# wyf0912/ContextGS

Measured on AMD Instinct MI355X. Metric: views/sec fwd+bwd @1920×1080, 1M anchors, higher is better.
Workload: dtype f32

## Files before the change

contextgs_amd/csrc/mlp3.hip:

```cpp
#include "cgs_internal.h"
#include "mlp_frag.h"
#include "buf_access.h"

#define M3_IN 54
#define M3_HID 50
#define M3_NTI 4
#define M3_XP 64
#define M3_NT1 4
#define M3_HP 64
#define M3_HCAT 150
#define M3_HLD 150
#define M3_HPITCH 50
#define M3_GLD 192
#define M3_GPITCH 64
#define M3_XLD 54
#ifndef M3_FWD_RT
#define M3_FWD_RT 1
#define M3_FWD_WAVES 16
#endif
#define M3_FWD_PATCH (16 * 70)
#ifndef M3_BWD_RT
#define M3_BWD_RT 2
#define M3_BWD_WAVES 8
#endif

#define M3_FENCE()                         \
    do {                                   \
        asm volatile("" ::: "memory");     \
        __builtin_amdgcn_sched_barrier(0); \
    } while (0)

struct M3Head {
    const float *W1, *b1, *W2, *b2;
    float *Y;
    const float *dY;
    float *dZ2;
};

template <int OUT>
struct M3FwdLds {
    static constexpr int NT2 = (OUT + 15) / 16, OP = NT2 * 16;
    static constexpr int S1 = frag_pad4mod8(M3_HP), S2 = frag_pad4mod8(OP);
    static constexpr int FLOATS = M3_XP * S1 + M3_HP * S2 + M3_HP + OP;
};

template <int OUT>
__device__ __forceinline__ void m3_stage_fwd(float *lds, const M3Head &h, int tid, int nthr) {
    using L = M3FwdLds<OUT>;
    float *W1s = lds, *W2s = W1s + M3_XP * L::S1, *b1s = W2s + M3_HP * L::S2, *b2s = b1s + M3_HP;
    frag_stage_transposed<M3_IN, M3_HID, M3_XP, L::S1>(W1s, h.W1, tid, nthr);
    frag_stage_transposed<M3_HID, OUT, M3_HP, L::S2>(W2s, h.W2, tid, nthr);
    for (int i = tid; i < M3_HP; i += nthr) b1s[i] = i < M3_HID ? h.b1[i] : 0.f;
    for (int i = tid; i < L::OP; i += nthr) b2s[i] = i < OUT ? h.b2[i] : 0.f;
}

#define M3_MAX_ROWS (4ll << 20)
struct M3FwdBufs { ClBuf H, Y[3], Xo, X, src, feat, anc; };

template <int OUT, int ACT, int RT, bool TILED, bool TM>
__device__ __forceinline__ void m3_head_fwd(const float *lds, const M3Head &h, int head, const f32x4 (&xb)[RT][M3_NTI],
                                            const bool (&valid)[RT], int64_t row0, int g, int c,
                                            float *__restrict__ Hcat, const M3FwdBufs &B, float *patch) {
    using L = M3FwdLds<OUT>;
    const float *W1s = lds, *W2s = W1s + M3_XP * L::S1, *b1s = W2s + M3_HP * L::S2, *b2s = b1s + M3_HP;
    f32x4 acc1[M3_NT1][RT];
#pragma unroll
    for (int t = 0; t < M3_NT1; ++t)
#pragma unroll
        for (int rt = 0; rt < RT; ++rt) acc1[t][rt] = (f32x4){0.f, 0.f, 0.f, 0.f};
#pragma unroll
    for (int q = 0; q < M3_NTI; ++q)
#pragma unroll
        for (int j = 0; j < 4; ++j) {
            if (16 * q + j >= M3_IN) continue;
            if (TM && q == M3_NTI - 1 && 16 * q + 4 * j >= M3_IN) continue;
#pragma unroll
            for (int t = 0; t < M3_NT1; ++t) {
                const float a = W1s[((TM && q == M3_NTI - 1) ? 16 * q + g + 4 * j : 16 * q + 4 * g + j) * L::S1 + 16 * t + c];
#pragma unroll
                for (int rt = 0; rt < RT; ++rt) acc1[t][rt] = frag_mfma(a, xb[rt][q][j], acc1[t][rt]);
            }
        }
#pragma unroll
    for (int t = 0; t < M3_NT1; ++t)
#pragma unroll
        for (int rt = 0; rt < RT; ++rt) {
            const int64_t row = row0 + rt * 16 + c;
#pragma unroll
            for (int r = 0; r < 4; ++r) acc1[t][rt][r] = fmaxf(acc1[t][rt][r] + b1s[16 * t + 4 * g + r], 0.f);
            if (TILED)
                frag_tstore4<M3_HID>(B.H, (uint32_t)((row0 + rt * 16) >> 4) * (16 * M3_HLD * 4) + (uint32_t)head * (16 * M3_HID * 4), t, g, c,
                                     valid[rt], acc1[t][rt]);
            else
                frag_bstore4<M3_HID>(B.H, (uint32_t)row * (M3_HLD * 4) + (uint32_t)(M3_HPITCH * head) * 4, t, g, valid[rt], acc1[t][rt]);
        }
    f32x4 acc2[L::NT2][RT];
#pragma unroll
    for (int u = 0; u < L::NT2; ++u)
#pragma unroll
        for (int rt = 0; rt < RT; ++rt) acc2[u][rt] = (f32x4){0.f, 0.f, 0.f, 0.f};
#pragma unroll
    for (int t = 0; t < M3_NT1; ++t)
#pragma unroll
        for (int r = 0; r < 4; ++r) {
            if (16 * t + r >= M3_HID) continue;
#pragma unroll
            for (int u = 0; u < L::NT2; ++u) {
                const float a = W2s[(16 * t + 4 * g + r) * L::S2 + 16 * u + c];
#pragma unroll
                for (int rt = 0; rt < RT; ++rt) acc2[u][rt] = frag_mfma(a, acc1[t][rt][r], acc2[u][rt]);
            }
        }
#pragma unroll
    for (int rt = 0; rt < RT; ++rt) {
        f32x4 yv[L::NT2];
#pragma unroll
        for (int u = 0; u < L::NT2; ++u)
#pragma unroll
            for (int r = 0; r < 4; ++r) yv[u][r] = frag_act<ACT>(acc2[u][rt][r] + b2s[16 * u + 4 * g + r]);
        frag_tile_store<OUT, L::NT2>(patch, B.Y[head], (uint32_t)(row0 + rt * 16) * (OUT * 4), yv, g, c, 16 * g + c);
    }
}

struct M3Rows {
    const float *feat_src;
    const int64_t *src_row;
    const float *anchor;
    const float *cam;
    float *X_out;
    float *d_feat_src;
    float *d_anchor;
};

template <bool TM = false>
__device__ __forceinline__ f32x4 m3_load_x_rows_b(const M3FwdBufs &B, float cam0, float cam1, float cam2, int64_t row, int64_t srow,
                                                  int q, int g, bool valid) {
    const uint32_t fo = (uint32_t)srow * (M3_HID * 4);
    if (q < 3) return cl_l128(B.feat, cl_sel(valid, fo + (uint32_t)(16 * q + 4 * g) * 4));
    if (TM) {
        const f32x4 f2 = cl_l64(B.feat, cl_sel(valid && g < 2, fo + 48 * 4));
        const f32x4 a = cl_l96(B.anc, cl_sel(valid, (uint32_t)row * 12));
        const float ux = a[0] - cam0, uy = a[1] - cam1, uz = a[2] - cam2;
        const float dist = sqrtf(ux * ux + uy * uy + uz * uz);
        const float s0 = g == 0 ? f2[0] : (g == 1 ? f2[1] : (g == 2 ? ux / dist : uy / dist));
        const float s1 = g == 0 ? uz / dist : (g == 1 ? dist : 0.f);
        return valid ? (f32x4){s0, s1, 0.f, 0.f} : (f32x4){0.f, 0.f, 0.f, 0.f};
    }
    const f32x4 f2 = cl_l64(B.feat, cl_sel(valid && g == 0, fo + 48 * 4));
    const f32x4 a = cl_l96(B.anc, cl_sel(valid && g < 2, (uint32_t)row * 12));
    const float ux = a[0] - cam0, uy = a[1] - cam1, uz = a[2] - cam2;
    const float dist = sqrtf(ux * ux + uy * uy + uz * uz);
    const f32x4 v0 = (f32x4){f2[0], f2[1], ux / dist, uy / dist}, v1 = (f32x4){uz / dist, dist, 0.f, 0.f};
    const f32x4 z = (f32x4){0.f, 0.f, 0.f, 0.f};
    return !valid ? z : (g == 0 ? v0 : (g == 1 ? v1 : z));
}

template <int O0, int A0, int O1, int A1, int O2, int A2, int RT, int WAVES, bool ROWS, bool TILED = false>
__global__ void __launch_bounds__(WAVES * 64)
    mlp3_fwd_kernel(const float *__restrict__ X, int64_t ldx, M3Head h0, M3Head h1, M3Head h2,
                    float *__restrict__ Hcat, int64_t n, M3Rows R) {
    constexpr int WFL = M3FwdLds<O0>::FLOATS + M3FwdLds<O1>::FLOATS + M3FwdLds<O2>::FLOATS;
    static_assert(WFL % 4 == 0 && O0 <= 70 && O1 <= 70 && O2 <= 70 && M3_IN <= 70, "patch: 16-byte aligned, the widest image fits");
    __shared__ __attribute__((aligned(16))) float lds[WFL + WAVES * M3_FWD_PATCH];
    float *l0 = lds, *l1 = l0 + M3FwdLds<O0>::FLOATS, *l2 = l1 + M3FwdLds<O1>::FLOATS;
    const int tid = threadIdx.x, nthr = WAVES * 64;
    float *patch = lds + WFL + (tid >> 6) * M3_FWD_PATCH;
    m3_stage_fwd<O0>(l0, h0, tid, nthr);
    m3_stage_fwd<O1>(l1, h1, tid, nthr);
    m3_stage_fwd<O2>(l2, h2, tid, nthr);
    __syncthreads();
    const int lane = tid & 63, wave = tid >> 6, g = lane >> 4, c = lane & 15;
    const int64_t ntiles = (n + 16 * RT - 1) / (16 * RT);
    f32x4 xb[RT][M3_NTI], xn[RT][M3_NTI];
    bool valid[RT], validn[RT];
    const int64_t tile0 = (int64_t)blockIdx.x * WAVES + wave, tstride = (int64_t)gridDim.x * WAVES;
    M3FwdBufs B;
    {
        const uint64_t nb = (uint64_t)n;
        const uint64_t nbt = (nb + 15) / 16 * 16;
        B.H = cl_buf(Hcat, (TILED ? nbt : nb) * (M3_HLD * 4));
        B.Y[0] = cl_buf(h0.Y, nb * (O0 * 4)); B.Y[1] = cl_buf(h1.Y, nb * (O1 * 4)); B.Y[2] = cl_buf(h2.Y, nb * (O2 * 4));
        B.Xo = cl_buf(ROWS ? R.X_out : nullptr, nb * (M3_XLD * 4));
        B.X = cl_buf(ROWS ? nullptr : X, nb > 0 ? ((nb - 1) * (uint64_t)ldx + M3_IN) * 4 : 0);
        B.src = cl_buf(ROWS ? R.src_row : nullptr, nb * 8);
        B.feat = cl_buf(ROWS ? R.feat_src : nullptr, CL_MAX_BYTES);
        B.anc = cl_buf(ROWS ? R.anchor : nullptr, nb * 12);
    }
    const float cam0 = ROWS ? R.cam[0] : 0.f, cam1 = ROWS ? R.cam[1] : 0.f, cam2 = ROWS ? R.cam[2] : 0.f;
    const uint32_t ldx4 = (uint32_t)ldx * 4;
    int64_t srow_n[RT], srow_nn[RT];
#pragma unroll
    for (int rt = 0; rt < RT; ++rt) {
        const int64_t row = tile0 * 16 * RT + rt * 16 + c, rown = row + tstride * 16 * RT;
        valid[rt] = tile0 < ntiles && row < n;
        const int64_t srow = ROWS ? cl_li64(B.src, cl_sel(valid[rt], (uint32_t)row * 8)) : 0;
        srow_n[rt] = ROWS ? cl_li64(B.src, cl_sel(rown < n, (uint32_t)rown * 8)) : 0;
#pragma unroll
        for (int q = 0; q < M3_NTI; ++q)
            xb[rt][q] = ROWS ? m3_load_x_rows_b<true>(B, cam0, cam1, cam2, row, srow, q, g, valid[rt])
                             : frag_bmask4<M3_IN>(frag_bload4<M3_IN>(B.X, (uint32_t)row * ldx4, q, g, valid[rt]), q, g);
    }
    for (int64_t tile = tile0; tile < ntiles; tile += tstride) {
        const int64_t row0 = tile * 16 * RT;
        asm volatile("" ::: "memory");
#pragma unroll
        for (int rt = 0; rt < RT; ++rt) {
            const int64_t row = (tile + tstride) * 16 * RT + rt * 16 + c, rownn = row + tstride * 16 * RT;
            validn[rt] = row < n;
            srow_nn[rt] = ROWS ? cl_li64(B.src, cl_sel(rownn < n, (uint32_t)rownn * 8)) : 0;
#pragma unroll
            for (int q = 0; q < M3_NTI; ++q)
                xn[rt][q] = ROWS ? m3_load_x_rows_b<true>(B, cam0, cam1, cam2, row, srow_n[rt], q, g, validn[rt])
                                 : frag_bmask4<M3_IN>(frag_bload4<M3_IN>(B.X, (uint32_t)row * ldx4, q, g, validn[rt]), q, g);
        }
        if (ROWS) {
#pragma unroll
            for (int rt = 0; rt < RT; ++rt)
                if (R.X_out) {
#pragma unroll
                    for (int q = 0; q < M3_NTI - 1; ++q) cl_patch_put4(patch + c * M3_IN + 16 * q + 4 * g, xb[rt][q], 4);
                    patch[c * M3_IN + 48 + g] = xb[rt][M3_NTI - 1][0];
                    if (g < 2) patch[c * M3_IN + 52 + g] = xb[rt][M3_NTI - 1][1];
                    cl_patch_flush<64 * M3_IN>(patch, B.Xo, (uint32_t)(row0 + rt * 16) * (M3_XLD * 4), lane);
                }
        }
        m3_head_fwd<O0, A0, RT, TILED, ROWS>(l0, h0, 0, xb, valid, row0, g, c, Hcat, B, patch);
        m3_head_fwd<O1, A1, RT, TILED, ROWS>(l1, h1, 1, xb, valid, row0, g, c, Hcat, B, patch);
        m3_head_fwd<O2, A2, RT, TILED, ROWS>(l2, h2, 2, xb, valid, row0, g, c, Hcat, B, patch);
#pragma unroll
        for (int rt = 0; rt < RT; ++rt) {
            valid[rt] = validn[rt];
            srow_n[rt] = srow_nn[rt];
#pragma unroll
            for (int q = 0; q < M3_NTI; ++q) xb[rt][q] = xn[rt][q];
        }
    }
}

template <int OUT>
struct M3BwdLds {
    static constexpr int NT2 = (OUT + 15) / 16, OP = NT2 * 16;
    static constexpr int SA = frag_pad4mod8(M3_HP), SB = frag_pad4mod8(M3_XP);
    static constexpr int FLOATS = OP * SA + M3_HP * SB;
};

template <int OUT>
__device__ __forceinline__ void m3_stage_bwd(float *lds, const M3Head &h, int tid, int nthr) {
    using L = M3BwdLds<OUT>;
    float *W2n = lds, *W1n = W2n + L::OP * L::SA;
    frag_stage_loop(h.W2, L::OP * L::SA, tid, nthr,
                    [](int i) { const int o = i / L::SA, hh = i % L::SA; return (o < OUT && hh < M3_HID) ? o * M3_HID + hh : -1; },
                    [&](int i, float v) { W2n[i] = v; });
    frag_stage_loop(h.W1, M3_HP * L::SB, tid, nthr,
                    [](int i) { const int hh = i / L::SB, k = i % L::SB; return (hh < M3_HID && k < M3_IN) ? hh * M3_IN + k : -1; },
                    [&](int i, float v) { W1n[i] = v; });
}

template <int OUT, int ACT, int RT>
__device__ __forceinline__ void m3_head_bwd(const float *lds, const M3Head &h, int head, const bool (&valid)[RT],
                                            int64_t row0, int g, int c, const float *__restrict__ Hcat,
                                            float *__restrict__ dZ1cat, f32x4 (&adx)[M3_NTI][RT]) {
    using L = M3BwdLds<OUT>;
    const float *W2n = lds, *W1n = W2n + L::OP * L::SA;
    f32x4 adh[M3_NT1][RT];
#pragma unroll
    for (int t = 0; t < M3_NT1; ++t)
#pragma unroll
        for (int rt = 0; rt < RT; ++rt) adh[t][rt] = (f32x4){0.f, 0.f, 0.f, 0.f};
    f32x4 b[L::NT2][RT], yv[L::NT2][RT], hv[M3_NT1][RT];
#pragma unroll
    for (int u = 0; u < L::NT2; ++u)
#pragma unroll
        for (int rt = 0; rt < RT; ++rt) {
            const int64_t row = row0 + rt * 16 + c;
            b[u][rt] = frag_load4<OUT>(h.dY + row * OUT, u, g, valid[rt]);
            if (ACT != FRAG_ACT_NONE) yv[u][rt] = frag_load4<OUT>(h.Y + row * OUT, u, g, valid[rt]);
        }
#pragma unroll
    for (int t = 0; t < M3_NT1; ++t)
#pragma unroll
        for (int rt = 0; rt < RT; ++rt)
            hv[t][rt] = frag_load4<M3_HID>(Hcat + (row0 + rt * 16 + c) * M3_HLD + M3_HPITCH * head, t, g, valid[rt]);
    if (ACT != FRAG_ACT_NONE) {
#pragma unroll
        for (int u = 0; u < L::NT2; ++u)
#pragma unroll
            for (int rt = 0; rt < RT; ++rt) {
#pragma unroll
                for (int r = 0; r < 4; ++r) b[u][rt][r] *= frag_act_grad<ACT>(yv[u][rt][r]);
                frag_store4<OUT>(h.dZ2 + (row0 + rt * 16 + c) * OUT, u, g, valid[rt], b[u][rt]);
            }
    }
#pragma unroll
    for (int u = 0; u < L::NT2; ++u)
#pragma unroll
        for (int j = 0; j < 4; ++j) {
            if (16 * u + j >= OUT) continue;
#pragma unroll
            for (int t = 0; t < M3_NT1; ++t) {
                const float a = W2n[(16 * u + 4 * g + j) * L::SA + 16 * t + c];
#pragma unroll
                for (int rt = 0; rt < RT; ++rt) adh[t][rt] = frag_mfma(a, b[u][rt][j], adh[t][rt]);
            }
        }
#pragma unroll
    for (int t = 0; t < M3_NT1; ++t)
#pragma unroll
        for (int rt = 0; rt < RT; ++rt) {
            const int64_t at = (row0 + rt * 16 + c) * M3_GLD + M3_GPITCH * head;
#pragma unroll
            for (int r = 0; r < 4; ++r) adh[t][rt][r] = hv[t][rt][r] > 0.f ? adh[t][rt][r] : 0.f;
            frag_store4<M3_HP>(dZ1cat + at, t, g, valid[rt], adh[t][rt]);
        }
#pragma unroll
    for (int t = 0; t < M3_NT1; ++t)
#pragma unroll
        for (int r = 0; r < 4; ++r) {
            if (16 * t + r >= M3_HID) continue;
#pragma unroll
            for (int v = 0; v < M3_NTI; ++v) {
                const float a = W1n[(16 * t + 4 * g + r) * L::SB + 16 * v + c];
#pragma unroll
                for (int rt = 0; rt < RT; ++rt) adx[v][rt] = frag_mfma(a, adh[t][rt][r], adx[v][rt]);
            }
        }
}

template <int O0, int A0, int O1, int A1, int O2, int A2, int RT, int WAVES, bool ROWS>
__global__ void __launch_bounds__(WAVES * 64)
    mlp3_bwd_kernel(M3Head h0, M3Head h1, M3Head h2, const float *__restrict__ Hcat, float *__restrict__ dZ1cat,
                    float *__restrict__ dX, int64_t lddx, int64_t n, M3Rows R) {
    __shared__ float lds[M3BwdLds<O0>::FLOATS + M3BwdLds<O1>::FLOATS + M3BwdLds<O2>::FLOATS];
    float *l0 = lds, *l1 = l0 + M3BwdLds<O0>::FLOATS, *l2 = l1 + M3BwdLds<O1>::FLOATS;
    const int tid = threadIdx.x, nthr = WAVES * 64;
    m3_stage_bwd<O0>(l0, h0, tid, nthr);
    m3_stage_bwd<O1>(l1, h1, tid, nthr);
    m3_stage_bwd<O2>(l2, h2, tid, nthr);
    __syncthreads();
    const int lane = tid & 63, wave = tid >> 6, g = lane >> 4, c = lane & 15;
    const int64_t ntiles = (n + 16 * RT - 1) / (16 * RT);
    for (int64_t tile = (int64_t)blockIdx.x * WAVES + wave; tile < ntiles; tile += (int64_t)gridDim.x * WAVES) {
        const int64_t row0 = tile * 16 * RT;
        asm volatile("" ::: "memory");
        bool valid[RT];
#pragma unroll
        for (int rt = 0; rt < RT; ++rt) valid[rt] = row0 + rt * 16 + c < n;
        f32x4 adx[M3_NTI][RT];
#pragma unroll
        for (int v = 0; v < M3_NTI; ++v)
#pragma unroll
            for (int rt = 0; rt < RT; ++rt) adx[v][rt] = (f32x4){0.f, 0.f, 0.f, 0.f};
        m3_head_bwd<O0, A0, RT>(l0, h0, 0, valid, row0, g, c, Hcat, dZ1cat, adx);
        m3_head_bwd<O1, A1, RT>(l1, h1, 1, valid, row0, g, c, Hcat, dZ1cat, adx);
        m3_head_bwd<O2, A2, RT>(l2, h2, 2, valid, row0, g, c, Hcat, dZ1cat, adx);
        if (ROWS) {
#pragma unroll
            for (int rt = 0; rt < RT; ++rt) {
                const int64_t row = row0 + rt * 16 + c;
                const int64_t srow = valid[rt] ? R.src_row[row] : 0;
                float *dst = R.d_feat_src + srow * M3_HID;
#pragma unroll
                for (int v = 0; v < 3; ++v)
                    if (valid[rt]) *(f32x4_a4 *)(dst + 16 * v + 4 * g) = adx[v][rt];
                const float z52 = __shfl(adx[3][rt][0], 16 + c, 64), z53 = __shfl(adx[3][rt][1], 16 + c, 64);
                if (g == 0 && valid[rt]) {
                    dst[48] = adx[3][rt][0];
                    dst[49] = adx[3][rt][1];
                    const float dvx = adx[3][rt][2], dvy = adx[3][rt][3], dvz = z52, dd = z53;
                    const float ux = R.anchor[3 * row] - R.cam[0], uy = R.anchor[3 * row + 1] - R.cam[1],
                                uz = R.anchor[3 * row + 2] - R.cam[2];
                    const float dist = sqrtf(ux * ux + uy * uy + uz * uz), inv = 1.f / dist;
                    const float vx = ux * inv, vy = uy * inv, vz = uz * inv;
                    const float dot = vx * dvx + vy * dvy + vz * dvz;
                    R.d_anchor[3 * row] = (dvx - vx * dot) * inv + vx * dd;
                    R.d_anchor[3 * row + 1] = (dvy - vy * dot) * inv + vy * dd;
                    R.d_anchor[3 * row + 2] = (dvz - vz * dot) * inv + vz * dd;
                }
            }
        } else if (dX) {
#pragma unroll
            for (int v = 0; v < M3_NTI; ++v)
#pragma unroll
                for (int rt = 0; rt < RT; ++rt)
                    frag_store4<M3_IN>(dX + (row0 + rt * 16 + c) * lddx, v, g, valid[rt], adx[v][rt]);
        }
    }
}


#define M3W_LD 20
#define M3W_PATCH (16 * M3W_LD)
#define M3W_NPATCH 13
#define M3W_WAVES 4
#define M3W_E (M3_GLD * (M3_IN + 1) + (10 + 30 + 70) * (M3_HID + 1))

__device__ __forceinline__ f32x4 m3w_f2n(float *patch, f32x4 v, int g, int c) {
    *(f32x4 *)(patch + c * M3W_LD + 4 * g) = v;
    f32x4 o;
#pragma unroll
    for (int r = 0; r < 4; ++r) o[r] = patch[(4 * g + r) * M3W_LD + c];
    return o;
}

struct M3wBufs { ClBuf dY[3], Y[3], H, X; };
template <int OUT, int ACT>
struct M3wOps {
    static constexpr int NT2 = (OUT + 15) / 16;
    f32x4 dy[NT2], y[ACT != FRAG_ACT_NONE ? NT2 : 1], h[M3_NT1];
    template <bool TILED = false>
    __device__ __forceinline__ void load(const M3wBufs &B, int head, int64_t row, int g, bool valid) {
        const uint32_t ro = (uint32_t)row * (OUT * 4), rh = (uint32_t)row * (M3_HLD * 4) + (uint32_t)(M3_HPITCH * head) * 4;
        const uint32_t th = (uint32_t)(row >> 4) * (16 * M3_HLD * 4) + (uint32_t)head * (16 * M3_HID * 4);
#pragma unroll
        for (int u = 0; u < NT2; ++u) {
            dy[u] = frag_bload4<OUT>(B.dY[head], ro, u, g, valid);
            if (ACT != FRAG_ACT_NONE) y[u] = frag_bload4<OUT>(B.Y[head], ro, u, g, valid);
        }
#pragma unroll
        for (int t = 0; t < M3_NT1; ++t)
            h[t] = TILED ? frag_tload4<M3_HID>(B.H, th, t, g, (int)(row & 15), valid) : frag_bload4<M3_HID>(B.H, rh, t, g, valid);
    }
    __device__ __forceinline__ void mask(int g) {
#pragma unroll
        for (int u = 0; u < NT2; ++u) {
            dy[u] = frag_bmask4<OUT>(dy[u], u, g);
            if (ACT != FRAG_ACT_NONE) y[u] = frag_bmask4<OUT>(y[u], u, g);
        }
#pragma unroll
        for (int t = 0; t < M3_NT1; ++t) h[t] = frag_bmask4<M3_HID>(h[t], t, g);
    }
};

__device__ __forceinline__ void m3w_put(float *patch, f32x4 v, int g, int c) { *(f32x4 *)(patch + c * M3W_LD + 4 * g) = v; }
__device__ __forceinline__ f32x4 m3w_get(const float *patch, int g, int c) {
    f32x4 o;
#pragma unroll
    for (int r = 0; r < 4; ++r) o[r] = patch[(4 * g + r) * M3W_LD + c];
    return o;
}

template <int OUT, int ACT, class Prefetch>
__device__ __forceinline__ void m3w_head(const float *lds, float *patches, M3wOps<OUT, ACT> &op, f32x4 ones, int g, int c,
                                         const f32x4 (&xn)[M3_NTI], f32x4 (&adx)[M3_NTI],
                                         f32x4 (&aw2)[(OUT + 15) / 16][M3_NT1], f32x4 (&aw1)[M3_NT1][M3_NTI], Prefetch prefetch) {
    using L = M3BwdLds<OUT>;
    const float *W2n = lds, *W1n = W2n + L::OP * L::SA;
    op.mask(g);
    f32x4 b[L::NT2];
#pragma unroll
    for (int u = 0; u < L::NT2; ++u) {
        b[u] = op.dy[u];
        if (ACT != FRAG_ACT_NONE) {
#pragma unroll
            for (int r = 0; r < 4; ++r) b[u][r] *= frag_act_grad<ACT>(op.y[u][r]);
        }
    }
#pragma unroll
    for (int t = 0; t < M3_NT1; ++t) m3w_put(patches + t * M3W_PATCH, op.h[t], g, c);
#pragma unroll
    for (int u = 0; u < L::NT2; ++u) m3w_put(patches + (4 + u) * M3W_PATCH, b[u], g, c);
    auto ldw2 = [&](int u, int j) {
        f32x4 w;
#pragma unroll
        for (int t = 0; t < M3_NT1; ++t) w[t] = W2n[(16 * u + 4 * g + j) * L::SA + 16 * t + c];
        return w;
    };
    auto ldw1 = [&](int t, int r) {
        f32x4 w;
#pragma unroll
        for (int v = 0; v < M3_NTI; ++v) w[v] = W1n[(16 * t + 4 * g + r) * L::SB + 16 * v + c];
        return w;
    };
    f32x4 adh[M3_NT1], hn[M3_NT1], zc;
#pragma unroll
    for (int t = 0; t < M3_NT1; ++t) adh[t] = (f32x4){0.f, 0.f, 0.f, 0.f};
    {
        f32x4 wc = ldw2(0, 0);
#pragma unroll
        for (int u = 0; u < L::NT2; ++u)
#pragma unroll
            for (int j = 0; j < 4; ++j) {
                if (16 * u + j >= OUT) continue;
                const int un = j == 3 ? u + 1 : u, jn = j == 3 ? 0 : j + 1;
                f32x4 wn = wc;
                if (un < L::NT2 && 16 * un + jn < OUT) wn = ldw2(un, jn);
                M3_FENCE();
#pragma unroll
                for (int t = 0; t < M3_NT1; ++t) adh[t] = frag_mfma(wc[t], b[u][j], adh[t]);
                M3_FENCE();
                wc = wn;
            }
    }
#pragma unroll
    for (int t = 0; t < M3_NT1; ++t) {
#pragma unroll
        for (int r = 0; r < 4; ++r) adh[t][r] = op.h[t][r] > 0.f ? adh[t][r] : 0.f;
        m3w_put(patches + (9 + t) * M3W_PATCH, adh[t], g, c);
    }
#pragma unroll
    for (int t = 0; t < M3_NT1; ++t) hn[t] = m3w_get(patches + t * M3W_PATCH, g, c);
    zc = m3w_get(patches + 4 * M3W_PATCH, g, c);
    if (c == M3_HID - 48) hn[3] = ones;
#pragma unroll
    for (int u = 0; u < L::NT2; ++u) {
        f32x4 zn = zc;
        if (u + 1 < L::NT2) zn = m3w_get(patches + (4 + u + 1) * M3W_PATCH, g, c);
        M3_FENCE();
#pragma unroll
        for (int r = 0; r < 4; ++r)
#pragma unroll
            for (int t = 0; t < M3_NT1; ++t) aw2[u][t] = frag_mfma(zc[r], hn[t][r], aw2[u][t]);
        M3_FENCE();
        zc = zn;
    }
    prefetch();
    f32x4 wx = ldw1(0, 0);
#pragma unroll
    for (int t = 0; t < M3_NT1; ++t)
#pragma unroll
        for (int r = 0; r < 4; ++r) {
            if (16 * t + r >= M3_HID) continue;
            const int tn = r == 3 ? t + 1 : t, rn = r == 3 ? 0 : r + 1;
            f32x4 wn = wx;
            if (tn < M3_NT1 && 16 * tn + rn < M3_HID) wn = ldw1(tn, rn);
            M3_FENCE();
#pragma unroll
            for (int v = 0; v < M3_NTI; ++v) adx[v] = frag_mfma(wx[v], adh[t][r], adx[v]);
            M3_FENCE();
            wx = wn;
        }
    f32x4 dc = m3w_get(patches + 9 * M3W_PATCH, g, c);
#pragma unroll
    for (int t = 0; t < M3_NT1; ++t) {
        f32x4 dn = dc;
        if (t + 1 < M3_NT1) dn = m3w_get(patches + (9 + t + 1) * M3W_PATCH, g, c);
        M3_FENCE();
#pragma unroll
        for (int r = 0; r < 4; ++r)
#pragma unroll
            for (int v = 0; v < M3_NTI; ++v) aw1[t][v] = frag_mfma(dc[r], xn[v][r], aw1[t][v]);
        M3_FENCE();
        dc = dn;
    }
}

template <bool ROWS, bool TL = false>
__global__ void __launch_bounds__(M3W_WAVES * 64) __attribute__((amdgpu_waves_per_eu(1, 1)))
    mlp3_bwd_wg_kernel(M3Head h0, M3Head h1, M3Head h2, const float *__restrict__ X, int64_t ldx,
                       const float *__restrict__ Hcat, float *__restrict__ dX, int64_t lddx, int64_t n, M3Rows R,
                       float *__restrict__ partial) {
    constexpr int WF = M3BwdLds<10>::FLOATS + M3BwdLds<30>::FLOATS + M3BwdLds<70>::FLOATS;
    constexpr int PF = M3W_WAVES * M3W_NPATCH * M3W_PATCH;
    static_assert(WF + PF >= M3W_E, "the LDS image of the weight gradients reuses the weight region");
    __shared__ __attribute__((aligned(16))) float lds[WF + PF];
    float *l0 = lds, *l1 = l0 + M3BwdLds<10>::FLOATS, *l2 = l1 + M3BwdLds<30>::FLOATS;
    const int tid = threadIdx.x, nthr = M3W_WAVES * 64;
    m3_stage_bwd<10>(l0, h0, tid, nthr);
    m3_stage_bwd<30>(l1, h1, tid, nthr);
    m3_stage_bwd<70>(l2, h2, tid, nthr);
    __syncthreads();
    const int lane = tid & 63, wave = tid >> 6, g = lane >> 4, c = lane & 15;
    float *patches = lds + WF + wave * M3W_NPATCH * M3W_PATCH;
    const int64_t ntiles = (n + 15) / 16;
    f32x4 a2_0[1][M3_NT1], a2_1[2][M3_NT1], a2_2[5][M3_NT1], a1_0[M3_NT1][M3_NTI], a1_1[M3_NT1][M3_NTI], a1_2[M3_NT1][M3_NTI];
    const f32x4 zero = (f32x4){0.f, 0.f, 0.f, 0.f};
#pragma unroll
    for (int t = 0; t < M3_NT1; ++t) {
        a2_0[0][t] = zero;
#pragma unroll
        for (int u = 0; u < 2; ++u) a2_1[u][t] = zero;
#pragma unroll
        for (int u = 0; u < 5; ++u) a2_2[u][t] = zero;
#pragma unroll
        for (int v = 0; v < M3_NTI; ++v) { a1_0[t][v] = zero; a1_1[t][v] = zero; a1_2[t][v] = zero; }
    }
    const int64_t tstride = (int64_t)gridDim.x * M3W_WAVES;
    int64_t tile = (int64_t)blockIdx.x * M3W_WAVES + wave;
    const uint64_t nb = (uint64_t)n;
    M3wBufs B;
    B.dY[0] = cl_buf(h0.dY, nb * 40); B.dY[1] = cl_buf(h1.dY, nb * 120); B.dY[2] = cl_buf(h2.dY, nb * 280);
    B.Y[0] = cl_buf(h0.Y, nb * 40); B.Y[1] = cl_buf(h1.Y, nb * 120); B.Y[2] = cl_buf(h2.Y, nb * 280);
    static_assert(ROWS || !TL, "the tiled hand-over belongs to the ROWS pair");
    B.H = cl_buf(Hcat, (TL ? (nb + 15) / 16 * 16 : nb) * (M3_HLD * 4));
    B.X = cl_buf(X, nb > 0 ? ((nb - 1) * (uint64_t)ldx + M3_IN) * 4 : 0);
    const ClBuf bSrc = cl_buf(ROWS ? R.src_row : nullptr, nb * 8), bAnc = cl_buf(ROWS ? R.anchor : nullptr, nb * 12);
    const float cam0 = ROWS ? R.cam[0] : 0.f, cam1 = ROWS ? R.cam[1] : 0.f, cam2 = ROWS ? R.cam[2] : 0.f;
    const uint32_t ldx4 = (uint32_t)ldx * 4;
    const bool regather = ROWS && X == nullptr;
    M3FwdBufs FB;
    FB.feat = cl_buf(regather ? R.feat_src : nullptr, CL_MAX_BYTES);
    FB.anc = bAnc;
    auto load_x = [&](f32x4 (&x)[M3_NTI], int64_t row, int64_t srow, bool v) {
#pragma unroll
        for (int q = 0; q < M3_NTI; ++q)
            x[q] = regather ? m3_load_x_rows_b(FB, cam0, cam1, cam2, row, srow, q, g, v)
                            : frag_bload4<M3_IN>(B.X, (uint32_t)row * ldx4, q, g, v);
    };
    M3wOps<10, 1> op0;
    M3wOps<30, 2> op1;
    M3wOps<70, 0> op2;
    f32x4 xf[M3_NTI];
    int64_t srow_next = 0;
    {
        const int64_t row = tile * 16 + c;
        const bool v0 = tile < ntiles && row < n;
        op0.template load<TL>(B, 0, row, g, v0);
        const int64_t s0 = regather ? cl_li64(bSrc, cl_sel(v0, (uint32_t)row * 8)) : 0;
        load_x(xf, row, s0, v0);
    }
    for (; tile < ntiles; tile += tstride) {
        const int64_t row0 = tile * 16;
        asm volatile("" ::: "memory");
        const bool valid = row0 + c < n;
        const int64_t rown = row0 + tstride * 16 + c;
        const bool validn = rown < n;
        f32x4 ones, xn[M3_NTI];
#pragma unroll
        for (int r = 0; r < 4; ++r) ones[r] = row0 + 4 * g + r < n ? 1.f : 0.f;
        const int64_t srow_pre = ROWS ? cl_li64(bSrc, cl_sel(valid, (uint32_t)(row0 + c) * 8)) : 0;
        if (regather) srow_next = cl_li64(bSrc, cl_sel(validn, (uint32_t)rown * 8));
        const f32x4 anc_pre = ROWS ? cl_l96(bAnc, cl_sel(valid && g == 0, (uint32_t)(row0 + c) * 12)) : zero;
#pragma unroll
        for (int q = 0; q < M3_NTI; ++q) m3w_put(patches + q * M3W_PATCH, frag_bmask4<M3_IN>(xf[q], q, g), g, c);
#pragma unroll
        for (int q = 0; q < M3_NTI; ++q) xn[q] = m3w_get(patches + q * M3W_PATCH, g, c);
        if (c == M3_IN - 48) xn[3] = ones;
        f32x4 adx[M3_NTI];
#pragma unroll
        for (int v = 0; v < M3_NTI; ++v) adx[v] = zero;
        m3w_head<10, 1>(l0, patches, op0, ones, g, c, xn, adx, a2_0, a1_0, [&]() { op1.template load<TL>(B, 1, row0 + c, g, valid); });
        m3w_head<30, 2>(l1, patches, op1, ones, g, c, xn, adx, a2_1, a1_1, [&]() { op2.template load<TL>(B, 2, row0 + c, g, valid); });
        m3w_head<70, 0>(l2, patches, op2, ones, g, c, xn, adx, a2_2, a1_2, [&]() {
            op0.template load<TL>(B, 0, rown, g, validn);
            load_x(xf, rown, srow_next, validn);
        });
        if (ROWS) {
            const int64_t row = row0 + c;
            const int64_t srow = valid ? srow_pre : 0;
            float *dst = R.d_feat_src + srow * M3_HID;
#pragma unroll
            for (int v = 0; v < 3; ++v)
                if (valid) *(f32x4_a4 *)(dst + 16 * v + 4 * g) = adx[v];
            const float z52 = __shfl(adx[3][0], 16 + c, 64), z53 = __shfl(adx[3][1], 16 + c, 64);
            if (g == 0 && valid) {
                dst[48] = adx[3][0];
                dst[49] = adx[3][1];
                const float dvx = adx[3][2], dvy = adx[3][3], dvz = z52, dd = z53;
                const float ux = anc_pre[0] - cam0, uy = anc_pre[1] - cam1, uz = anc_pre[2] - cam2;
                const float dist = sqrtf(ux * ux + uy * uy + uz * uz), inv = 1.f / dist;
                const float vx = ux * inv, vy = uy * inv, vz = uz * inv;
                const float dot = vx * dvx + vy * dvy + vz * dvz;
                R.d_anchor[3 * row] = (dvx - vx * dot) * inv + vx * dd;
                R.d_anchor[3 * row + 1] = (dvy - vy * dot) * inv + vy * dd;
                R.d_anchor[3 * row + 2] = (dvz - vz * dot) * inv + vz * dd;
            }
        } else if (dX) {
#pragma unroll
            for (int v = 0; v < M3_NTI; ++v) frag_store4<M3_IN>(dX + (row0 + c) * lddx, v, g, valid, adx[v]);
        }
    }
    __syncthreads();
    for (int i = tid; i < M3W_E; i += nthr) lds[i] = 0.f;
    __syncthreads();
    float *img1 = lds, *imgb1 = img1 + M3_GLD * M3_IN;
    for (int w = 0; w < M3W_WAVES; ++w) {
        if (wave == w) {
#pragma unroll
            for (int hd = 0; hd < 3; ++hd) {
                const f32x4 (&a1)[M3_NT1][M3_NTI] = hd == 0 ? a1_0 : (hd == 1 ? a1_1 : a1_2);
#pragma unroll
                for (int t = 0; t < M3_NT1; ++t)
#pragma unroll
                    for (int v = 0; v < M3_NTI; ++v)
#pragma unroll
                        for (int r = 0; r < 4; ++r) {
                            const int m = M3_GPITCH * hd + 16 * t + 4 * g + r, k = 16 * v + c;
                            if (k < M3_IN) img1[m * M3_IN + k] += a1[t][v][r];
                            else if (k == M3_IN) imgb1[m] += a1[t][v][r];
                        }
            }
            float *img2 = imgb1 + M3_GLD;
#define M3W_IMG2(ACC, NT2_, OUT_)                                                          \
            {                                                                               \
                _Pragma("unroll") for (int u = 0; u < NT2_; ++u)                            \
                _Pragma("unroll") for (int t = 0; t < M3_NT1; ++t)                          \
                _Pragma("unroll") for (int r = 0; r < 4; ++r) {                             \
                    const int o = 16 * u + 4 * g + r, hh = 16 * t + c;                      \
                    if (o < OUT_) {                                                         \
                        if (hh < M3_HID) img2[o * M3_HID + hh] += ACC[u][t][r];             \
                        else if (hh == M3_HID) img2[OUT_ * M3_HID + o] += ACC[u][t][r];     \
                    }                                                                       \
                }                                                                           \
                img2 += OUT_ * (M3_HID + 1);                                                \
            }
            M3W_IMG2(a2_0, 1, 10)
            M3W_IMG2(a2_1, 2, 30)
            M3W_IMG2(a2_2, 5, 70)
#undef M3W_IMG2
        }
        __syncthreads();
    }
    float *dstp = partial + (int64_t)blockIdx.x * M3W_E;
    for (int i = tid; i < M3W_E; i += nthr) dstp[i] = lds[i];
}


static int m3_cus() {
    static int cus = 0;
    if (!cus) {
        int dev = 0;
        hipDeviceProp_t p;
        if (hipGetDevice(&dev) == hipSuccess && hipGetDeviceProperties(&p, dev) == hipSuccess) cus = p.multiProcessorCount;
        if (cus <= 0) cus = 256;
    }
    return cus;
}

extern "C" int cgs_anchor_mlp3_layout(int *out4) {
    if (!out4) { cgs_set_error("cgs_anchor_mlp3_layout: NULL"); return CGS_ERR_ARG; }
    out4[0] = M3_HLD; out4[1] = M3_XLD; out4[2] = M3_GLD; out4[3] = M3_GPITCH;
    return CGS_OK;
}

extern "C" int cgs_anchor_mlp3_forward(const float *X, int64_t ldx, const float *const *W1, const float *const *b1,
                                       const float *const *W2, const float *const *b2, float *Y_op, float *Y_color,
                                       float *Y_cov, float *Hcat, int64_t n, void *stream) {
    if (n < 0) { cgs_set_error("anchor_mlp3_forward: n < 0"); return CGS_ERR_ARG; }
    if (n == 0) return CGS_OK;
    if (!X || !W1 || !b1 || !W2 || !b2 || !Y_op || !Y_color || !Y_cov) { cgs_set_error("anchor_mlp3_forward: NULL"); return CGS_ERR_ARG; }
    constexpr int RT = M3_FWD_RT, WAVES = M3_FWD_WAVES;
    M3Head h[3];
    float *ys[3] = {Y_op, Y_color, Y_cov};
    for (int i = 0; i < 3; ++i) h[i] = M3Head{W1[i], b1[i], W2[i], b2[i], ys[i], nullptr, nullptr};
    if (ldx < M3_IN || ldx > 4096) { cgs_set_error("anchor_mlp3_forward: ldx out of range"); return CGS_ERR_ARG; }
    CgsProfScope prof(CGS_PROF_MLP_FWD, (hipStream_t)stream);
    const int64_t step = ldx <= 256 ? M3_MAX_ROWS : M3_MAX_ROWS / 16;
    for (int64_t r0 = 0; r0 < n; r0 += step) {
        const int64_t m = n - r0 < step ? n - r0 : step;
        for (int i = 0; i < 3; ++i) h[i].Y = ys[i] + r0 * (i == 0 ? 10 : (i == 1 ? 30 : 70));
        const int64_t tiles = (m + 16 * RT - 1) / (16 * RT);
        const int64_t want = (tiles + WAVES - 1) / WAVES;
        const int grid = (int)(want < m3_cus() ? want : m3_cus());
        hipLaunchKernelGGL((mlp3_fwd_kernel<10, 1, 30, 2, 70, 0, RT, WAVES, false>), dim3(grid), dim3(WAVES * 64), 0, (hipStream_t)stream,
                           X + r0 * ldx, ldx, h[0], h[1], h[2], Hcat ? Hcat + r0 * M3_HLD : nullptr, m, M3Rows{});
    }
    CGS_CHECK_HIP(hipGetLastError());
    return CGS_OK;
}

extern "C" int cgs_anchor_mlp3_forward_rows_t(const float *feat_src, const int64_t *src_row, const float *anchor_vis,
                                              const float *cam3, float *X_out, const float *const *W1,
                                              const float *const *b1, const float *const *W2, const float *const *b2,
                                              float *Y_op, float *Y_color, float *Y_cov, float *Hcat, int64_t n, int tiled,
                                              void *stream);
extern "C" int cgs_anchor_mlp3_forward_rows(const float *feat_src, const int64_t *src_row, const float *anchor_vis,
                                            const float *cam3, float *X_out, const float *const *W1,
                                            const float *const *b1, const float *const *W2, const float *const *b2,
                                            float *Y_op, float *Y_color, float *Y_cov, float *Hcat, int64_t n, void *stream) {
    return cgs_anchor_mlp3_forward_rows_t(feat_src, src_row, anchor_vis, cam3, X_out, W1, b1, W2, b2, Y_op, Y_color, Y_cov, Hcat, n, 0,
                                          stream);
}
extern "C" int cgs_anchor_mlp3_forward_rows_t(const float *feat_src, const int64_t *src_row, const float *anchor_vis,
                                              const float *cam3, float *X_out, const float *const *W1,
                                              const float *const *b1, const float *const *W2, const float *const *b2,
                                              float *Y_op, float *Y_color, float *Y_cov, float *Hcat, int64_t n, int tiled,
                                              void *stream) {
    if (tiled && n > M3_MAX_ROWS) { cgs_set_error("anchor_mlp3_forward_rows: tiled hand-over needs <= %lld rows", (long long)M3_MAX_ROWS); return CGS_ERR_ARG; }
    if (n < 0) { cgs_set_error("anchor_mlp3_forward_rows: n < 0"); return CGS_ERR_ARG; }
    if (n == 0) return CGS_OK;
    if (!feat_src || !src_row || !anchor_vis || !cam3 || !W1 || !b1 || !W2 || !b2 || !Y_op || !Y_color || !Y_cov) {
        cgs_set_error("anchor_mlp3_forward_rows: NULL");
        return CGS_ERR_ARG;
    }
    constexpr int RT = M3_FWD_RT, WAVES = M3_FWD_WAVES;
    M3Head h[3];
    float *ys[3] = {Y_op, Y_color, Y_cov};
    for (int i = 0; i < 3; ++i) h[i] = M3Head{W1[i], b1[i], W2[i], b2[i], ys[i], nullptr, nullptr};
    CgsProfScope prof(CGS_PROF_MLP_FWD, (hipStream_t)stream);
    for (int64_t r0 = 0; r0 < n; r0 += M3_MAX_ROWS) {
        const int64_t m = n - r0 < M3_MAX_ROWS ? n - r0 : M3_MAX_ROWS;
        for (int i = 0; i < 3; ++i) h[i].Y = ys[i] + r0 * (i == 0 ? 10 : (i == 1 ? 30 : 70));
        const int64_t tiles = (m + 16 * RT - 1) / (16 * RT);
        const int64_t want = (tiles + WAVES - 1) / WAVES;
        const int grid = (int)(want < m3_cus() ? want : m3_cus());
        M3Rows R{feat_src, src_row + r0, anchor_vis + 3 * r0, cam3, X_out ? X_out + r0 * M3_XLD : nullptr, nullptr, nullptr};
        if (tiled)
            hipLaunchKernelGGL((mlp3_fwd_kernel<10, 1, 30, 2, 70, 0, RT, WAVES, true, true>), dim3(grid), dim3(WAVES * 64), 0, (hipStream_t)stream,
                               nullptr, 0, h[0], h[1], h[2], Hcat, m, R);
        else
            hipLaunchKernelGGL((mlp3_fwd_kernel<10, 1, 30, 2, 70, 0, RT, WAVES, true>), dim3(grid), dim3(WAVES * 64), 0, (hipStream_t)stream,
                               nullptr, 0, h[0], h[1], h[2], Hcat ? Hcat + r0 * M3_HLD : nullptr, m, R);
    }
    CGS_CHECK_HIP(hipGetLastError());
    return CGS_OK;
}

static int m3_backward(const float *X, int64_t ldx, const float *const *W1, const float *const *W2, const float *Y_op,
                       const float *Y_color, const float *dY_op, const float *dY_color, const float *dY_cov,
                       const float *Hcat, float *dX, int64_t lddx, float *dZ1cat, float *dZ2_op, float *dZ2_color,
                       float *dW1cat, float *db1cat, float *const *dW2, float *const *db2, int64_t n, void *scratch,
                       size_t scratch_bytes, const M3Rows *rows, void *stream_, int tiled = 0);
extern "C" int cgs_anchor_mlp3_wgrad(const float *X, int64_t ldx, const float *Hcat, const float *dZ1cat,
                                     const float *dZ2_op, const float *dZ2_color, const float *dY_cov, float *dW1cat,
                                     float *db1cat, float *const *dW2, float *const *db2, int64_t n, void *scratch,
                                     size_t scratch_bytes, void *stream_);

extern "C" int cgs_anchor_mlp3_backward(const float *X, int64_t ldx, const float *const *W1, const float *const *W2,
                                        const float *Y_op, const float *Y_color, const float *dY_op,
                                        const float *dY_color, const float *dY_cov, const float *Hcat, float *dX,
                                        int64_t lddx, float *dZ1cat, float *dZ2_op, float *dZ2_color, float *dW1cat,
                                        float *db1cat, float *const *dW2, float *const *db2, int64_t n, void *scratch,
                                        size_t scratch_bytes, void *stream_) {
    return m3_backward(X, ldx, W1, W2, Y_op, Y_color, dY_op, dY_color, dY_cov, Hcat, dX, lddx, dZ1cat, dZ2_op, dZ2_color,
                       dW1cat, db1cat, dW2, db2, n, scratch, scratch_bytes, nullptr, stream_);
}

extern "C" int cgs_anchor_mlp3_backward_rows_t(const float *X, const float *feat_src, const int64_t *src_row, const float *anchor_vis,
                                               const float *cam3, const float *const *W1, const float *const *W2,
                                               const float *Y_op, const float *Y_color, const float *dY_op,
                                               const float *dY_color, const float *dY_cov, const float *Hcat,
                                               float *d_feat_src, float *d_anchor_vis, float *dZ1cat, float *dZ2_op,
                                               float *dZ2_color, float *dW1cat, float *db1cat, float *const *dW2,
                                               float *const *db2, int64_t n, int tiled, void *scratch, size_t scratch_bytes,
                                               void *stream_);
extern "C" int cgs_anchor_mlp3_backward_rows(const float *X, const float *feat_src, const int64_t *src_row, const float *anchor_vis,
                                             const float *cam3, const float *const *W1, const float *const *W2,
                                             const float *Y_op, const float *Y_color, const float *dY_op,
                                             const float *dY_color, const float *dY_cov, const float *Hcat,
                                             float *d_feat_src, float *d_anchor_vis, float *dZ1cat, float *dZ2_op,
                                             float *dZ2_color, float *dW1cat, float *db1cat, float *const *dW2,
                                             float *const *db2, int64_t n, void *scratch, size_t scratch_bytes,
                                             void *stream_) {
    return cgs_anchor_mlp3_backward_rows_t(X, feat_src, src_row, anchor_vis, cam3, W1, W2, Y_op, Y_color, dY_op, dY_color, dY_cov, Hcat,
// ... 112 lines not shown
```

Before: 159.8.

## Pack the two leftover hidden units of all three heads into one shared MFMA tile

Each head's hidden layer of 50 units was padded to four 16-wide MFMA tiles, which wastes most of the fourth tile. The change computes the first 48 units per head in three tiles. The remaining 2 units of each head are packed into a single shared tail tile that holds 4 columns per head, used in forward layer 1, in the layer-2 contribution and in the backward weight-gradient accumulation. This cuts MFMA work and accumulator registers, at the cost of extra indexing, an extra LDS staging region and lane-dependent selects.

After: 161.6 (median of 6 runs). 1.01x the previous value.

```diff
diff --git a/contextgs_amd/csrc/mlp3.hip b/contextgs_amd/csrc/mlp3.hip
--- a/contextgs_amd/csrc/mlp3.hip
+++ b/contextgs_amd/csrc/mlp3.hip
@@ -9,6 +9,14 @@
 #define M3_NT1 4
 #define M3_HP 64
 #define M3_HCAT 150
+#define M3_NTF 3
+#define M3_HF 48
+#define M3_NTP 10
+#define M3_TS 20
+__host__ __device__ constexpr int m3_packed_col(int head, int unit) {
+    return unit < M3_HF ? M3_HF * head + unit : 3 * M3_HF + 4 * head + (unit - M3_HF);
+}
+static_assert(m3_packed_col(2, 47) == 143 && m3_packed_col(0, 48) == 144 && m3_packed_col(2, 49) == 16 * M3_NTP - 7, "ten tiles");
 #define M3_HLD 150
 #define M3_HPITCH 50
 #define M3_GLD 192
@@ -40,49 +48,92 @@
 template <int OUT>
 struct M3FwdLds {
     static constexpr int NT2 = (OUT + 15) / 16, OP = NT2 * 16;
-    static constexpr int S1 = frag_pad4mod8(M3_HP), S2 = frag_pad4mod8(OP);
-    static constexpr int FLOATS = M3_XP * S1 + M3_HP * S2 + M3_HP + OP;
+    static constexpr int S1 = frag_pad4mod8(M3_HF), S2 = frag_pad4mod8(OP);
+    static constexpr int FLOATS = M3_XP * S1 + M3_HP * S2 + M3_HF + OP;
 };
+#define M3_TAIL_FLOATS (M3_XP * M3_TS + 16)
 
 template <int OUT>
 __device__ __forceinline__ void m3_stage_fwd(float *lds, const M3Head &h, int tid, int nthr) {
     using L = M3FwdLds<OUT>;
-    float *W1s = lds, *W2s = W1s + M3_XP * L::S1, *b1s = W2s + M3_HP * L::S2, *b2s = b1s + M3_HP;
-    frag_stage_transposed<M3_IN, M3_HID, M3_XP, L::S1>(W1s, h.W1, tid, nthr);
+    float *W1s = lds, *W2s = W1s + M3_XP * L::S1, *b1s = W2s + M3_HP * L::S2, *b2s = b1s + M3_HF;
+    frag_stage_transposed<M3_IN, M3_HF, M3_XP, L::S1>(W1s, h.W1, tid, nthr);
     frag_stage_transposed<M3_HID, OUT, M3_HP, L::S2>(W2s, h.W2, tid, nthr);
-    for (int i = tid; i < M3_HP; i += nthr) b1s[i] = i < M3_HID ? h.b1[i] : 0.f;
+    for (int i = tid; i < M3_HF; i += nthr) b1s[i] = h.b1[i];
     for (int i = tid; i < L::OP; i += nthr) b2s[i] = i < OUT ? h.b2[i] : 0.f;
+}
+__device__ __forceinline__ void m3_stage_fwd_tail(float *lds, const M3Head &h0, const M3Head &h1, const M3Head &h2, int tid, int nthr) {
+    for (int i = tid; i < M3_TAIL_FLOATS; i += nthr) {
+        const bool bias = i >= M3_XP * M3_TS;
+        const int k = i / M3_TS, col = bias ? i - M3_XP * M3_TS : i % M3_TS, hd = col >> 2, e = col & 3;
+        const M3Head &h = hd == 0 ? h0 : (hd == 1 ? h1 : h2);
+        float v = 0.f;
+        if (hd < 3 && e < M3_HID - M3_HF) {
+            if (bias) v = h.b1[M3_HF + e];
+            else if (k < M3_IN) v = h.W1[(M3_HF + e) * M3_IN + k];
+        }
+        lds[i] = v;
+    }
 }
 
 #define M3_MAX_ROWS (4ll << 20)
 struct M3FwdBufs { ClBuf H, Y[3], Xo, X, src, feat, anc; };
 
-template <int OUT, int ACT, int RT, bool TILED, bool TM>
-__device__ __forceinline__ void m3_head_fwd(const float *lds, const M3Head &h, int head, const f32x4 (&xb)[RT][M3_NTI],
-                                            const bool (&valid)[RT], int64_t row0, int g, int c,
-                                            float *__restrict__ Hcat, const M3FwdBufs &B, float *patch) {
-    using L = M3FwdLds<OUT>;
-    const float *W1s = lds, *W2s = W1s + M3_XP * L::S1, *b1s = W2s + M3_HP * L::S2, *b2s = b1s + M3_HP;
-    f32x4 acc1[M3_NT1][RT];
-#pragma unroll
-    for (int t = 0; t < M3_NT1; ++t)
-#pragma unroll
-        for (int rt = 0; rt < RT; ++rt) acc1[t][rt] = (f32x4){0.f, 0.f, 0.f, 0.f};
+template <int RT, bool TILED, bool TM>
+__device__ __forceinline__ void m3_tail_fwd(const float *lds, const f32x4 (&xb)[RT][M3_NTI], const bool (&valid)[RT], int64_t row0,
+                                            int g, int c, const M3FwdBufs &B, f32x4 (&acct)[RT]) {
+    const float *W1t = lds, *b1t = W1t + M3_XP * M3_TS;
+#pragma unroll
+    for (int rt = 0; rt < RT; ++rt) acct[rt] = (f32x4){0.f, 0.f, 0.f, 0.f};
 #pragma unroll
     for (int q = 0; q < M3_NTI; ++q)
 #pragma unroll
         for (int j = 0; j < 4; ++j) {
             if (16 * q + j >= M3_IN) continue;
             if (TM && q == M3_NTI - 1 && 16 * q + 4 * j >= M3_IN) continue;
-#pragma unroll
-            for (int t = 0; t < M3_NT1; ++t) {
+            const float a = W1t[((TM && q == M3_NTI - 1) ? 16 * q + g + 4 * j : 16 * q + 4 * g + j) * M3_TS + c];
+#pragma unroll
+            for (int rt = 0; rt < RT; ++rt) acct[rt] = frag_mfma(a, xb[rt][q][j], acct[rt]);
+        }
+#pragma unroll
+    for (int rt = 0; rt < RT; ++rt) {
+        const int64_t row = row0 + rt * 16 + c;
+#pragma unroll
+        for (int r = 0; r < 4; ++r) acct[rt][r] = fmaxf(acct[rt][r] + b1t[4 * g + r], 0.f);
+        if (TILED)
+            cl_s64(B.H, cl_sel(valid[rt] && g < 3, (uint32_t)((row0 + rt * 16) >> 4) * (16 * M3_HLD * 4) + (uint32_t)g * (16 * M3_HID * 4) +
+                                                       frag_toff<M3_HID>(M3_NTF, 0, c)), acct[rt]);
+        else
+            cl_s64(B.H, cl_sel(valid[rt] && g < 3, (uint32_t)row * (M3_HLD * 4) + (uint32_t)(M3_HPITCH * g + M3_HF) * 4), acct[rt]);
+    }
+}
+
+template <int OUT, int ACT, int RT, bool TILED, bool TM>
+__device__ __forceinline__ void m3_head_fwd(const float *lds, const M3Head &h, int head, const f32x4 (&xb)[RT][M3_NTI],
+                                            const f32x4 (&acct)[RT], const bool (&valid)[RT], int64_t row0, int g, int c,
+                                            float *__restrict__ Hcat, const M3FwdBufs &B, float *patch) {
+    using L = M3FwdLds<OUT>;
+    const float *W1s = lds, *W2s = W1s + M3_XP * L::S1, *b1s = W2s + M3_HP * L::S2, *b2s = b1s + M3_HF;
+    f32x4 acc1[M3_NTF][RT];
+#pragma unroll
+    for (int t = 0; t < M3_NTF; ++t)
+#pragma unroll
+        for (int rt = 0; rt < RT; ++rt) acc1[t][rt] = (f32x4){0.f, 0.f, 0.f, 0.f};
+#pragma unroll
+    for (int q = 0; q < M3_NTI; ++q)
+#pragma unroll
+        for (int j = 0; j < 4; ++j) {
+            if (16 * q + j >= M3_IN) continue;
+            if (TM && q == M3_NTI - 1 && 16 * q + 4 * j >= M3_IN) continue;
+#pragma unroll
+            for (int t = 0; t < M3_NTF; ++t) {
                 const float a = W1s[((TM && q == M3_NTI - 1) ? 16 * q + g + 4 * j : 16 * q + 4 * g + j) * L::S1 + 16 * t + c];
 #pragma unroll
                 for (int rt = 0; rt < RT; ++rt) acc1[t][rt] = frag_mfma(a, xb[rt][q][j], acc1[t][rt]);
             }
         }
 #pragma unroll
-    for (int t = 0; t < M3_NT1; ++t)
+    for (int t = 0; t < M3_NTF; ++t)
 #pragma unroll
         for (int rt = 0; rt < RT; ++rt) {
             const int64_t row = row0 + rt * 16 + c;
@@ -100,10 +151,9 @@
 #pragma unroll
         for (int rt = 0; rt < RT; ++rt) acc2[u][rt] = (f32x4){0.f, 0.f, 0.f, 0.f};
 #pragma unroll
-    for (int t = 0; t < M3_NT1; ++t)
+    for (int t = 0; t < M3_NTF; ++t)
 #pragma unroll
         for (int r = 0; r < 4; ++r) {
-            if (16 * t + r >= M3_HID) continue;
 #pragma unroll
             for (int u = 0; u < L::NT2; ++u) {
                 const float a = W2s[(16 * t + 4 * g + r) * L::S2 + 16 * u + c];
@@ -111,6 +161,15 @@
                 for (int rt = 0; rt < RT; ++rt) acc2[u][rt] = frag_mfma(a, acc1[t][rt][r], acc2[u][rt]);
             }
         }
+#pragma unroll
+    for (int r = 0; r < M3_HID - M3_HF; ++r) {
+#pragma unroll
+        for (int u = 0; u < L::NT2; ++u) {
+            const float a = W2s[(M3_HF + 4 * ((g - head) & 3) + r) * L::S2 + 16 * u + c];
+#pragma unroll
+            for (int rt = 0; rt < RT; ++rt) acc2[u][rt] = frag_mfma(a, g == head ? acct[rt][r] : 0.f, acc2[u][rt]);
+        }
+    }
 #pragma unroll
     for (int rt = 0; rt < RT; ++rt) {
         f32x4 yv[L::NT2];
@@ -159,15 +218,16 @@
 __global__ void __launch_bounds__(WAVES * 64)
     mlp3_fwd_kernel(const float *__restrict__ X, int64_t ldx, M3Head h0, M3Head h1, M3Head h2,
                     float *__restrict__ Hcat, int64_t n, M3Rows R) {
-    constexpr int WFL = M3FwdLds<O0>::FLOATS + M3FwdLds<O1>::FLOATS + M3FwdLds<O2>::FLOATS;
+    constexpr int WFL = M3FwdLds<O0>::FLOATS + M3FwdLds<O1>::FLOATS + M3FwdLds<O2>::FLOATS + M3_TAIL_FLOATS;
     static_assert(WFL % 4 == 0 && O0 <= 70 && O1 <= 70 && O2 <= 70 && M3_IN <= 70, "patch: 16-byte aligned, the widest image fits");
     __shared__ __attribute__((aligned(16))) float lds[WFL + WAVES * M3_FWD_PATCH];
-    float *l0 = lds, *l1 = l0 + M3FwdLds<O0>::FLOATS, *l2 = l1 + M3FwdLds<O1>::FLOATS;
+    float *l0 = lds, *l1 = l0 + M3FwdLds<O0>::FLOATS, *l2 = l1 + M3FwdLds<O1>::FLOATS, *lt = l2 + M3FwdLds<O2>::FLOATS;
     const int tid = threadIdx.x, nthr = WAVES * 64;
     float *patch = lds + WFL + (tid >> 6) * M3_FWD_PATCH;
     m3_stage_fwd<O0>(l0, h0, tid, nthr);
     m3_stage_fwd<O1>(l1, h1, tid, nthr);
     m3_stage_fwd<O2>(l2, h2, tid, nthr);
+    m3_stage_fwd_tail(lt, h0, h1, h2, tid, nthr);
     __syncthreads();
     const int lane = tid & 63, wave = tid >> 6, g = lane >> 4, c = lane & 15;
     const int64_t ntiles = (n + 16 * RT - 1) / (16 * RT);
@@ -224,9 +284,11 @@
                     cl_patch_flush<64 * M3_IN>(patch, B.Xo, (uint32_t)(row0 + rt * 16) * (M3_XLD * 4), lane);
                 }
         }
-        m3_head_fwd<O0, A0, RT, TILED, ROWS>(l0, h0, 0, xb, valid, row0, g, c, Hcat, B, patch);
-        m3_head_fwd<O1, A1, RT, TILED, ROWS>(l1, h1, 1, xb, valid, row0, g, c, Hcat, B, patch);
-        m3_head_fwd<O2, A2, RT, TILED, ROWS>(l2, h2, 2, xb, valid, row0, g, c, Hcat, B, patch);
+        f32x4 acct[RT];
+        m3_tail_fwd<RT, TILED, ROWS>(lt, xb, valid, row0, g, c, B, acct);
+        m3_head_fwd<O0, A0, RT, TILED, ROWS>(l0, h0, 0, xb, acct, valid, row0, g, c, Hcat, B, patch);
+        m3_head_fwd<O1, A1, RT, TILED, ROWS>(l1, h1, 1, xb, acct, valid, row0, g, c, Hcat, B, patch);
+        m3_head_fwd<O2, A2, RT, TILED, ROWS>(l2, h2, 2, xb, acct, valid, row0, g, c, Hcat, B, patch);
 #pragma unroll
         for (int rt = 0; rt < RT; ++rt) {
             valid[rt] = validn[rt];
@@ -439,10 +501,11 @@
     return o;
 }
 
-template <int OUT, int ACT, class Prefetch>
+template <int OUT, int ACT, int HEAD, class Prefetch>
 __device__ __forceinline__ void m3w_head(const float *lds, float *patches, M3wOps<OUT, ACT> &op, f32x4 ones, int g, int c,
                                          const f32x4 (&xn)[M3_NTI], f32x4 (&adx)[M3_NTI],
-                                         f32x4 (&aw2)[(OUT + 15) / 16][M3_NT1], f32x4 (&aw1)[M3_NT1][M3_NTI], Prefetch prefetch) {
+                                         f32x4 (&aw2)[(OUT + 15) / 16][M3_NT1], f32x4 (&aw1)[M3_NTF][M3_NTI],
+                                         f32x4 (&aw1t)[M3_NTI], Prefetch prefetch) {
     using L = M3BwdLds<OUT>;
     const float *W2n = lds, *W1n = W2n + L::OP * L::SA;
     op.mask(g);
@@ -495,7 +558,8 @@
     for (int t = 0; t < M3_NT1; ++t) {
 #pragma unroll
         for (int r = 0; r < 4; ++r) adh[t][r] = op.h[t][r] > 0.f ? adh[t][r] : 0.f;
-        m3w_put(patches + (9 + t) * M3W_PATCH, adh[t], g, c);
+        if (t < M3_NTF) m3w_put(patches + (9 + t) * M3W_PATCH, adh[t], g, c);
+        else *(f32x4 *)(patches + 12 * M3W_PATCH + c * M3W_LD + (g == 0 ? 4 * HEAD : 12)) = adh[t];
     }
 #pragma unroll
     for (int t = 0; t < M3_NT1; ++t) hn[t] = m3w_get(patches + t * M3W_PATCH, g, c);
@@ -529,16 +593,20 @@
             M3_FENCE();
             wx = wn;
         }
+    constexpr int NTD = HEAD == 2 ? M3_NTF + 1 : M3_NTF;
     f32x4 dc = m3w_get(patches + 9 * M3W_PATCH, g, c);
 #pragma unroll
-    for (int t = 0; t < M3_NT1; ++t) {
+    for (int t = 0; t < NTD; ++t) {
         f32x4 dn = dc;
-        if (t + 1 < M3_NT1) dn = m3w_get(patches + (9 + t + 1) * M3W_PATCH, g, c);
+        if (t + 1 < NTD) dn = m3w_get(patches + (9 + t + 1) * M3W_PATCH, g, c);
         M3_FENCE();
 #pragma unroll
         for (int r = 0; r < 4; ++r)
 #pragma unroll
-            for (int v = 0; v < M3_NTI; ++v) aw1[t][v] = frag_mfma(dc[r], xn[v][r], aw1[t][v]);
+            for (int v = 0; v < M3_NTI; ++v) {
+                if (t < M3_NTF) aw1[t][v] = frag_mfma(dc[r], xn[v][r], aw1[t][v]);
+                else aw1t[v] = frag_mfma(dc[r], xn[v][r], aw1t[v]);
+            }
         M3_FENCE();
         dc = dn;
     }
@@ -562,7 +630,7 @@
     const int lane = tid & 63, wave = tid >> 6, g = lane >> 4, c = lane & 15;
     float *patches = lds + WF + wave * M3W_NPATCH * M3W_PATCH;
     const int64_t ntiles = (n + 15) / 16;
-    f32x4 a2_0[1][M3_NT1], a2_1[2][M3_NT1], a2_2[5][M3_NT1], a1_0[M3_NT1][M3_NTI], a1_1[M3_NT1][M3_NTI], a1_2[M3_NT1][M3_NTI];
+    f32x4 a2_0[1][M3_NT1], a2_1[2][M3_NT1], a2_2[5][M3_NT1], a1_0[M3_NTF][M3_NTI], a1_1[M3_NTF][M3_NTI], a1_2[M3_NTF][M3_NTI], a1_t[M3_NTI];
     const f32x4 zero = (f32x4){0.f, 0.f, 0.f, 0.f};
 #pragma unroll
     for (int t = 0; t < M3_NT1; ++t) {
@@ -571,8 +639,13 @@
         for (int u = 0; u < 2; ++u) a2_1[u][t] = zero;
 #pragma unroll
         for (int u = 0; u < 5; ++u) a2_2[u][t] = zero;
-#pragma unroll
-        for (int v = 0; v < M3_NTI; ++v) { a1_0[t][v] = zero; a1_1[t][v] = zero; a1_2[t][v] = zero; }
+        if (t < M3_NTF) {
+#pragma unroll
+            for (int v = 0; v < M3_NTI; ++v) { a1_0[t][v] = zero; a1_1[t][v] = zero; a1_2[t][v] = zero; }
+        } else {
+#pragma unroll
+            for (int v = 0; v < M3_NTI; ++v) a1_t[v] = zero;
+        }
     }
     const int64_t tstride = (int64_t)gridDim.x * M3W_WAVES;
     int64_t tile = (int64_t)blockIdx.x * M3W_WAVES + wave;
@@ -628,9 +701,9 @@
         f32x4 adx[M3_NTI];
 #pragma unroll
         for (int v = 0; v < M3_NTI; ++v) adx[v] = zero;
-        m3w_head<10, 1>(l0, patches, op0, ones, g, c, xn, adx, a2_0, a1_0, [&]() { op1.template load<TL>(B, 1, row0 + c, g, valid); });
-        m3w_head<30, 2>(l1, patches, op1, ones, g, c, xn, adx, a2_1, a1_1, [&]() { op2.template load<TL>(B, 2, row0 + c, g, valid); });
-        m3w_head<70, 0>(l2, patches, op2, ones, g, c, xn, adx, a2_2, a1_2, [&]() {
+        m3w_head<10, 1, 0>(l0, patches, op0, ones, g, c, xn, adx, a2_0, a1_0, a1_t, [&]() { op1.template load<TL>(B, 1, row0 + c, g, valid); });
+        m3w_head<30, 2, 1>(l1, patches, op1, ones, g, c, xn, adx, a2_1, a1_1, a1_t, [&]() { op2.template load<TL>(B, 2, row0 + c, g, valid); });
+        m3w_head<70, 0, 2>(l2, patches, op2, ones, g, c, xn, adx, a2_2, a1_2, a1_t, [&]() {
             op0.template load<TL>(B, 0, rown, g, validn);
             load_x(xf, rown, srow_next, validn);
         });
@@ -667,9 +740,9 @@
         if (wave == w) {
 #pragma unroll
             for (int hd = 0; hd < 3; ++hd) {
-                const f32x4 (&a1)[M3_NT1][M3_NTI] = hd == 0 ? a1_0 : (hd == 1 ? a1_1 : a1_2);
-#pragma unroll
-                for (int t = 0; t < M3_NT1; ++t)
+                const f32x4 (&a1)[M3_NTF][M3_NTI] = hd == 0 ? a1_0 : (hd == 1 ? a1_1 : a1_2);
+#pragma unroll
+                for (int t = 0; t < M3_NTF; ++t)
 #pragma unroll
                     for (int v = 0; v < M3_NTI; ++v)
 #pragma unroll
@@ -679,6 +752,14 @@
                             else if (k == M3_IN) imgb1[m] += a1[t][v][r];
                         }
             }
+#pragma unroll
+            for (int v = 0; v < M3_NTI; ++v)
+#pragma unroll
+                for (int r = 0; r < M3_HID - M3_HF; ++r) {
+                    const int m = M3_GPITCH * g + M3_HF + r, k = 16 * v + c;
+                    if (g < 3 && k < M3_IN) img1[m * M3_IN + k] += a1_t[v][r];
+                    else if (g < 3 && k == M3_IN) imgb1[m] += a1_t[v][r];
+                }
             float *img2 = imgb1 + M3_GLD;
 #define M3W_IMG2(ACC, NT2_, OUT_)                                                          \
             {                                                                               \
```
